# Xiuyu-Li/q-diffusion

Measured on NVIDIA H100. Metric: images_per_sec, higher is better.
Workload: dtype int8 (W4/W8 codes x A8 codes, int32 accumulate; fp32 norms/softmax)

## Files before the change

q-diffusion_b200/csrc/attention_wg.cuh:

```cuda
#pragma once
#include "attention.cuh"
#include "ptx.cuh"

namespace qd {

__device__ __forceinline__ void wgmma_ra_s8s8_n64(uint32_t* d, const uint32_t (&a)[4], uint64_t db, uint32_t scale_d) {
  asm volatile(
      "{\n\t.reg .pred p;\n\t"
      "setp.ne.b32 p, %37, 0;\n\t"
      "wgmma.mma_async.sync.aligned.m64n64k32.s32.s8.s8 "
      "{%0, %1, %2, %3, %4, %5, %6, %7, %8, %9, %10, %11, %12, %13, %14, %15, %16, %17, %18, %19, %20, %21, %22, %23, %24, %25, %26, %27, %28, %29, %30, %31}, {%32, %33, %34, %35}, %36, p;\n\t}\n"
      : "+r"(d[0]), "+r"(d[1]), "+r"(d[2]), "+r"(d[3]), "+r"(d[4]), "+r"(d[5]), "+r"(d[6]), "+r"(d[7]), "+r"(d[8]), "+r"(d[9]), "+r"(d[10]), "+r"(d[11]), "+r"(d[12]), "+r"(d[13]), "+r"(d[14]), "+r"(d[15]), "+r"(d[16]), "+r"(d[17]), "+r"(d[18]), "+r"(d[19]), "+r"(d[20]), "+r"(d[21]), "+r"(d[22]), "+r"(d[23]), "+r"(d[24]), "+r"(d[25]), "+r"(d[26]), "+r"(d[27]), "+r"(d[28]), "+r"(d[29]), "+r"(d[30]), "+r"(d[31])
      : "r"(a[0]), "r"(a[1]), "r"(a[2]), "r"(a[3]), "l"(db), "r"(scale_d));
}
__device__ __forceinline__ void wgmma_ra_u8u8_n64(uint32_t* d, const uint32_t (&a)[4], uint64_t db, uint32_t scale_d) {
  asm volatile(
      "{\n\t.reg .pred p;\n\t"
      "setp.ne.b32 p, %37, 0;\n\t"
      "wgmma.mma_async.sync.aligned.m64n64k32.s32.u8.u8 "
      "{%0, %1, %2, %3, %4, %5, %6, %7, %8, %9, %10, %11, %12, %13, %14, %15, %16, %17, %18, %19, %20, %21, %22, %23, %24, %25, %26, %27, %28, %29, %30, %31}, {%32, %33, %34, %35}, %36, p;\n\t}\n"
      : "+r"(d[0]), "+r"(d[1]), "+r"(d[2]), "+r"(d[3]), "+r"(d[4]), "+r"(d[5]), "+r"(d[6]), "+r"(d[7]), "+r"(d[8]), "+r"(d[9]), "+r"(d[10]), "+r"(d[11]), "+r"(d[12]), "+r"(d[13]), "+r"(d[14]), "+r"(d[15]), "+r"(d[16]), "+r"(d[17]), "+r"(d[18]), "+r"(d[19]), "+r"(d[20]), "+r"(d[21]), "+r"(d[22]), "+r"(d[23]), "+r"(d[24]), "+r"(d[25]), "+r"(d[26]), "+r"(d[27]), "+r"(d[28]), "+r"(d[29]), "+r"(d[30]), "+r"(d[31])
      : "r"(a[0]), "r"(a[1]), "r"(a[2]), "r"(a[3]), "l"(db), "r"(scale_d));
}
__device__ __forceinline__ void wgmma_ra_f16_n64(float* d, const uint32_t (&a)[4], uint64_t db, uint32_t scale_d) {
// ... 97 lines not shown
}
__device__ __forceinline__ void wgmma_ra_u8s8_n96(uint32_t* d, const uint32_t (&a)[4], uint64_t db, uint32_t scale_d) {
  asm volatile(
      "{\n\t.reg .pred p;\n\t"
      "setp.ne.b32 p, %53, 0;\n\t"
      "wgmma.mma_async.sync.aligned.m64n96k32.s32.u8.s8 "
      "{%0, %1, %2, %3, %4, %5, %6, %7, %8, %9, %10, %11, %12, %13, %14, %15, %16, %17, %18, %19, %20, %21, %22, %23, %24, %25, %26, %27, %28, %29, %30, %31, %32, %33, %34, %35, %36, %37, %38, %39, %40, %41, %42, %43, %44, %45, %46, %47}, {%48, %49, %50, %51}, %52, p;\n\t}\n"
      : "+r"(d[0]), "+r"(d[1]), "+r"(d[2]), "+r"(d[3]), "+r"(d[4]), "+r"(d[5]), "+r"(d[6]), "+r"(d[7]), "+r"(d[8]), "+r"(d[9]), "+r"(d[10]), "+r"(d[11]), "+r"(d[12]), "+r"(d[13]), "+r"(d[14]), "+r"(d[15]), "+r"(d[16]), "+r"(d[17]), "+r"(d[18]), "+r"(d[19]), "+r"(d[20]), "+r"(d[21]), "+r"(d[22]), "+r"(d[23]), "+r"(d[24]), "+r"(d[25]), "+r"(d[26]), "+r"(d[27]), "+r"(d[28]), "+r"(d[29]), "+r"(d[30]), "+r"(d[31]), "+r"(d[32]), "+r"(d[33]), "+r"(d[34]), "+r"(d[35]), "+r"(d[36]), "+r"(d[37]), "+r"(d[38]), "+r"(d[39]), "+r"(d[40]), "+r"(d[41]), "+r"(d[42]), "+r"(d[43]), "+r"(d[44]), "+r"(d[45]), "+r"(d[46]), "+r"(d[47])
      : "r"(a[0]), "r"(a[1]), "r"(a[2]), "r"(a[3]), "l"(db), "r"(scale_d));
}
__device__ __forceinline__ void wgmma_ra_u8u8_n112(uint32_t* d, const uint32_t (&a)[4], uint64_t db, uint32_t scale_d) {
  asm volatile(
      "{\n\t.reg .pred p;\n\t"
      "setp.ne.b32 p, %61, 0;\n\t"
      "wgmma.mma_async.sync.aligned.m64n112k32.s32.u8.u8 "
      "{%0, %1, %2, %3, %4, %5, %6, %7, %8, %9, %10, %11, %12, %13, %14, %15, %16, %17, %18, %19, %20, %21, %22, %23, %24, %25, %26, %27, %28, %29, %30, %31, %32, %33, %34, %35, %36, %37, %38, %39, %40, %41, %42, %43, %44, %45, %46, %47, %48, %49, %50, %51, %52, %53, %54, %55}, {%56, %57, %58, %59}, %60, p;\n\t}\n"
      : "+r"(d[0]), "+r"(d[1]), "+r"(d[2]), "+r"(d[3]), "+r"(d[4]), "+r"(d[5]), "+r"(d[6]), "+r"(d[7]), "+r"(d[8]), "+r"(d[9]), "+r"(d[10]), "+r"(d[11]), "+r"(d[12]), "+r"(d[13]), "+r"(d[14]), "+r"(d[15]), "+r"(d[16]), "+r"(d[17]), "+r"(d[18]), "+r"(d[19]), "+r"(d[20]), "+r"(d[21]), "+r"(d[22]), "+r"(d[23]), "+r"(d[24]), "+r"(d[25]), "+r"(d[26]), "+r"(d[27]), "+r"(d[28]), "+r"(d[29]), "+r"(d[30]), "+r"(d[31]), "+r"(d[32]), "+r"(d[33]), "+r"(d[34]), "+r"(d[35]), "+r"(d[36]), "+r"(d[37]), "+r"(d[38]), "+r"(d[39]), "+r"(d[40]), "+r"(d[41]), "+r"(d[42]), "+r"(d[43]), "+r"(d[44]), "+r"(d[45]), "+r"(d[46]), "+r"(d[47]), "+r"(d[48]), "+r"(d[49]), "+r"(d[50]), "+r"(d[51]), "+r"(d[52]), "+r"(d[53]), "+r"(d[54]), "+r"(d[55])
      : "r"(a[0]), "r"(a[1]), "r"(a[2]), "r"(a[3]), "l"(db), "r"(scale_d));
}
__device__ __forceinline__ void wgmma_ra_u8s8_n112(uint32_t* d, const uint32_t (&a)[4], uint64_t db, uint32_t scale_d) {
  asm volatile(
      "{\n\t.reg .pred p;\n\t"
      "setp.ne.b32 p, %61, 0;\n\t"
      "wgmma.mma_async.sync.aligned.m64n112k32.s32.u8.s8 "
      "{%0, %1, %2, %3, %4, %5, %6, %7, %8, %9, %10, %11, %12, %13, %14, %15, %16, %17, %18, %19, %20, %21, %22, %23, %24, %25, %26, %27, %28, %29, %30, %31, %32, %33, %34, %35, %36, %37, %38, %39, %40, %41, %42, %43, %44, %45, %46, %47, %48, %49, %50, %51, %52, %53, %54, %55}, {%56, %57, %58, %59}, %60, p;\n\t}\n"
      : "+r"(d[0]), "+r"(d[1]), "+r"(d[2]), "+r"(d[3]), "+r"(d[4]), "+r"(d[5]), "+r"(d[6]), "+r"(d[7]), "+r"(d[8]), "+r"(d[9]), "+r"(d[10]), "+r"(d[11]), "+r"(d[12]), "+r"(d[13]), "+r"(d[14]), "+r"(d[15]), "+r"(d[16]), "+r"(d[17]), "+r"(d[18]), "+r"(d[19]), "+r"(d[20]), "+r"(d[21]), "+r"(d[22]), "+r"(d[23]), "+r"(d[24]), "+r"(d[25]), "+r"(d[26]), "+r"(d[27]), "+r"(d[28]), "+r"(d[29]), "+r"(d[30]), "+r"(d[31]), "+r"(d[32]), "+r"(d[33]), "+r"(d[34]), "+r"(d[35]), "+r"(d[36]), "+r"(d[37]), "+r"(d[38]), "+r"(d[39]), "+r"(d[40]), "+r"(d[41]), "+r"(d[42]), "+r"(d[43]), "+r"(d[44]), "+r"(d[45]), "+r"(d[46]), "+r"(d[47]), "+r"(d[48]), "+r"(d[49]), "+r"(d[50]), "+r"(d[51]), "+r"(d[52]), "+r"(d[53]), "+r"(d[54]), "+r"(d[55])
      : "r"(a[0]), "r"(a[1]), "r"(a[2]), "r"(a[3]), "l"(db), "r"(scale_d));
}

constexpr int ATW_STAGES = 4;
constexpr int ATW_THREADS = ATT_WARPS * 32;
__host__ __device__ constexpr int atw_nv(int DV) {
  return DV + 8 <= 24 ? 24 : DV + 8 <= 32 ? 32 : DV + 8 <= 48 ? 48 : DV + 8 <= 64 ? 64 : DV + 8 <= 80 ? 80 : DV + 8 <= 96 ? 96 : 112;
}
struct AtwSmem {
  int k_bytes, v_bytes, z_off, bar_off, total;
};
__host__ __device__ inline AtwSmem atw_smem(int P, int NV) {
  AtwSmem l;
  l.k_bytes = (ATT_BN * P + 1023) / 1024 * 1024;
  l.v_bytes = (NV * ATT_BN + 1023) / 1024 * 1024;
  l.z_off = ATW_STAGES * (l.k_bytes + l.v_bytes);
  l.bar_off = l.z_off + ATW_STAGES * ATT_BN * 4;
  l.total = l.bar_off + ATW_STAGES * 8 + ATW_STAGES * 4 + 1024;
  return l;
}
__device__ __forceinline__ uint64_t atw_desc(uint32_t addr, int row_bytes) {
  const uint64_t layout = row_bytes == 128 ? 1 : row_bytes == 64 ? 2 : 3;
  uint64_t d = (uint64_t)((addr & 0x3FFFF) >> 4);
  d |= (uint64_t)1 << 16;
  d |= (uint64_t)((8 * row_bytes) >> 4) << 32;
  d |= layout << 62;
  return d;
}

template <int N, bool VS>
__device__ __forceinline__ void atw_pv(uint32_t* d, const uint32_t (&a)[4], uint64_t db, uint32_t scale_d) {
  if constexpr (VS) {
    if constexpr (N == 24) wgmma_ra_u8s8_n24(d, a, db, scale_d);
    else if constexpr (N == 32) wgmma_ra_u8s8_n32(d, a, db, scale_d);
    else if constexpr (N == 48) wgmma_ra_u8s8_n48(d, a, db, scale_d);
    else if constexpr (N == 64) wgmma_ra_u8s8_n64(d, a, db, scale_d);
    else if constexpr (N == 80) wgmma_ra_u8s8_n80(d, a, db, scale_d);
    else if constexpr (N == 96) wgmma_ra_u8s8_n96(d, a, db, scale_d);
    else wgmma_ra_u8s8_n112(d, a, db, scale_d);
  } else {
    if constexpr (N == 24) wgmma_ra_u8u8_n24(d, a, db, scale_d);
    else if constexpr (N == 32) wgmma_ra_u8u8_n32(d, a, db, scale_d);
    else if constexpr (N == 48) wgmma_ra_u8u8_n48(d, a, db, scale_d);
    else if constexpr (N == 64) wgmma_ra_u8u8_n64(d, a, db, scale_d);
    else if constexpr (N == 80) wgmma_ra_u8u8_n80(d, a, db, scale_d);
    else if constexpr (N == 96) wgmma_ra_u8u8_n96(d, a, db, scale_d);
    else wgmma_ra_u8u8_n112(d, a, db, scale_d);
  }
}

template <int DQ, int DV, bool QK_SIGNED, bool V_SIGNED, bool SM16, bool F16, int MINB>
__global__ void __launch_bounds__(ATW_THREADS, MINB)
qattention_wg_kernel(const __grid_constant__ CUtensorMap tmK, const __grid_constant__ CUtensorMap tmV,
                     const qd_attention_desc p, int P) {
  constexpr int NV = atw_nv(DV);
  constexpr int NKC = DQ / 32;
  constexpr int NDT = DV / 8 + 1;
  constexpr bool MAGIC = DV <= 64;
  constexpr int RB = F16 ? 2 * DV : DV;
  static_assert(!F16 || DV <= 64, "fp16 Q / K operands: d <= 64 keeps |S| below 2^22");
  using SV = att_score_t<F16>;
  extern __shared__ uint8_t atw_raw[];
  uint8_t* smem = atw_raw + (((smem_u32(atw_raw) + 1023u) & ~1023u) - smem_u32(atw_raw));
  const AtwSmem lay = atw_smem(P, NV);
  uint64_t* full = reinterpret_cast<uint64_t*>(smem + lay.bar_off);
  int* released = reinterpret_cast<int*>(full + ATW_STAGES);

  const int warp = threadIdx.x >> 5, lane = threadIdx.x & 31;
  const int g = lane >> 2, t = lane & 3;
  const int bh = blockIdx.y;
  const int b = bh / p.heads, h = bh - b * p.heads;
  const int row0 = blockIdx.x * ATT_BM + warp * 16;
  const int ntiles = (p.Tk + ATT_BN - 1) / ATT_BN;
  const int nloads = 2 * ntiles;
  const bool has_zq = !F16 && p.zq != 0;
  const int* zrk_g = reinterpret_cast<const int*>(p.ws) + (long long)bh * (long long)att_ws_stride(p.Tk);

  for (int i = threadIdx.x; i < ATW_STAGES * (NV - DV) * ATT_BN; i += ATW_THREADS) {
    const int s = i / ((NV - DV) * ATT_BN), r = (i / ATT_BN) % (NV - DV) + DV, c = i % ATT_BN;
    smem[ATW_STAGES * lay.k_bytes + s * lay.v_bytes + r * ATT_BN + c] = r == DV ? 1 : 0;
  }
  if (threadIdx.x == 0) {
    tma_prefetch_desc(&tmK);
    tma_prefetch_desc(&tmV);
    for (int s = 0; s < ATW_STAGES; ++s) {
      mbar_init(&full[s], 1);
      released[s] = 0;
    }
    fence_mbar_init();
  }
  fence_proxy_async();
  __syncthreads();

  auto issue = [&](int L) {
    const int s = L % ATW_STAGES, pass = L / ntiles, tile = L - pass * ntiles;
    const int j0 = tile * ATT_BN;
    const uint32_t bytes = (uint32_t)(ATT_BN * P) + (pass ? (uint32_t)(ATT_BN * DV) : 0u) + (has_zq ? ATT_BN * 4u : 0u);
    mbar_arrive_expect_tx(&full[s], bytes);
    tma_load_2d(smem + s * lay.k_bytes, &tmK, &full[s], h * P, b * p.Tk + j0);
    if (pass) tma_load_2d(smem + ATW_STAGES * lay.k_bytes + s * lay.v_bytes, &tmV, &full[s], j0, bh * DV);
    if (has_zq) bulk_load_1d(smem + lay.z_off + s * ATT_BN * 4, zrk_g + j0, ATT_BN * 4, &full[s]);
  };
  if (threadIdx.x == 0)
    for (int L = 0; L < ATW_STAGES && L < nloads; ++L) issue(L);

  constexpr bool QRELOAD = DV == 48;
  uint32_t qf[NKC][4];
  const uint8_t* qbase = reinterpret_cast<const uint8_t*>(p.q) + (long long)b * p.Tq * p.ld_q + p.q_off + h * p.head_stride_q;
  const uint8_t* q0 = qbase + (long long)min(row0 + g, p.Tq - 1) * p.ld_q;
  const uint8_t* q1 = qbase + (long long)min(row0 + g + 8, p.Tq - 1) * p.ld_q;
  auto load_q = [&]() {
#pragma unroll
    for (int kc = 0; kc < NKC; ++kc) {
      const int c0 = kc * 32 + 4 * t, c1 = c0 + 16;
      qf[kc][0] = c0 < RB ? *reinterpret_cast<const uint32_t*>(q0 + c0) : 0u;
      qf[kc][1] = c0 < RB ? *reinterpret_cast<const uint32_t*>(q1 + c0) : 0u;
      qf[kc][2] = c1 < RB ? *reinterpret_cast<const uint32_t*>(q0 + c1) : 0u;
      qf[kc][3] = c1 < RB ? *reinterpret_cast<const uint32_t*>(q1 + c1) : 0u;
    }
  };
  if constexpr (!QRELOAD) load_q();
  const float c = p.sim_scale * 1.4426950408889634f;
  const bool ragged = (p.Tk % ATT_BN) != 0;
  SV mi0 = att_lowest(SV{}), mi1 = att_lowest(SV{});
  float l0 = 0.f, l1 = 0.f;
  float off0 = 0.f, off1 = 0.f;
  uint32_t olo[NV / 2], ohi[SM16 ? NV / 2 : 1];
  const float pmax = (float)p.p_qmax;
  const QuantK oqk = make_quantk(p.oq);

  auto issue_s = [&](SV (&s)[8][4], int L) {
    const int st = L % ATW_STAGES;
    if constexpr (QRELOAD) load_q();
    mbar_wait(&full[st], (uint32_t)(L / ATW_STAGES) & 1u);
    const uint64_t dK = atw_desc(smem_u32(smem + st * lay.k_bytes), P);
    wgmma_fence();
#pragma unroll
    for (int kc = 0; kc < NKC; ++kc) {
      if constexpr (F16) wgmma_ra_f16_n64(&s[0][0], qf[kc], dK + (uint64_t)(2 * kc), kc ? 1u : 0u);
      else if constexpr (QK_SIGNED) wgmma_ra_s8s8_n64(reinterpret_cast<uint32_t*>(&s[0][0]), qf[kc], dK + (uint64_t)(2 * kc), kc ? 1u : 0u);
      else wgmma_ra_u8u8_n64(reinterpret_cast<uint32_t*>(&s[0][0]), qf[kc], dK + (uint64_t)(2 * kc), kc ? 1u : 0u);
    }
    wgmma_commit();
  };

  auto release = [&](int R) {
    __syncwarp();
    if (lane == 0) {
      const int s = R % ATW_STAGES;
      __threadfence_block();
      const int n = atomicAdd(&released[s], 1);
      if (n == ATT_WARPS * (R / ATW_STAGES + 1) - 1 && R + ATW_STAGES < nloads) {
        __threadfence_block();
        issue(R + ATW_STAGES);
      }
    }
  };

  auto softmax_pv = [&](SV (&sacc)[8][4], int L) {
    const int pass = L >= ntiles ? 1 : 0, tile = L - pass * ntiles, st = L % ATW_STAGES;
    const int j0 = tile * ATT_BN;
    if (L == ntiles) {
      l0 += __shfl_xor_sync(0xffffffffu, l0, 1);
      l0 += __shfl_xor_sync(0xffffffffu, l0, 2);
      l1 += __shfl_xor_sync(0xffffffffu, l1, 1);
      l1 += __shfl_xor_sync(0xffffffffu, l1, 2);
      off0 = -(float)mi0 * c + log2f(1.0f / (l0 * p.delta_w));
      off1 = -(float)mi1 * c + log2f(1.0f / (l1 * p.delta_w));
    }
    const int* sZrk = reinterpret_cast<const int*>(smem + lay.z_off + st * ATT_BN * 4);
    if (has_zq) {
#pragma unroll
      for (int nt = 0; nt < 8; ++nt) {
        const int2 z = *reinterpret_cast<const int2*>(sZrk + 8 * nt + 2 * t);
        sacc[nt][0] -= z.x; sacc[nt][1] -= z.y; sacc[nt][2] -= z.x; sacc[nt][3] -= z.y;
      }
    }
    if (ragged && tile == ntiles - 1) {
      const SV mask = att_mask<MAGIC>(SV{});
#pragma unroll
      for (int nt = 0; nt < 8; ++nt) {
        const int j = j0 + 8 * nt + 2 * t;
        if (j >= p.Tk) { sacc[nt][0] = mask; sacc[nt][2] = mask; }
        if (j + 1 >= p.Tk) { sacc[nt][1] = mask; sacc[nt][3] = mask; }
      }
    }
    if (pass == 0) {
      SV tm0 = sacc[0][0], tm1 = sacc[0][2];
#pragma unroll
      for (int nt = 0; nt < 8; ++nt) {
        tm0 = att_smax(tm0, att_smax(sacc[nt][0], sacc[nt][1]));
        tm1 = att_smax(tm1, att_smax(sacc[nt][2], sacc[nt][3]));
      }
      tm0 = att_smax(tm0, __shfl_xor_sync(0xffffffffu, tm0, 1));
      tm0 = att_smax(tm0, __shfl_xor_sync(0xffffffffu, tm0, 2));
      tm1 = att_smax(tm1, __shfl_xor_sync(0xffffffffu, tm1, 1));
      tm1 = att_smax(tm1, __shfl_xor_sync(0xffffffffu, tm1, 2));
      if (tm0 > mi0) { l0 *= (mi0 == att_lowest(SV{})) ? 0.f : ex2_approx((float)(mi0 - tm0) * c); mi0 = tm0; }
      if (tm1 > mi1) { l1 *= (mi1 == att_lowest(SV{})) ? 0.f : ex2_approx((float)(mi1 - tm1) * c); mi1 = tm1; }
      const float b0 = -(float)mi0 * c, b1 = -(float)mi1 * c;
      float a0 = 0.f, a1 = 0.f;
#pragma unroll
      for (int nt = 0; nt < 8; ++nt) {
        a0 += ex2_approx(fmaf(att_s2f<MAGIC>(sacc[nt][0]), c, b0)) + ex2_approx(fmaf(att_s2f<MAGIC>(sacc[nt][1]), c, b0));
        a1 += ex2_approx(fmaf(att_s2f<MAGIC>(sacc[nt][2]), c, b1)) + ex2_approx(fmaf(att_s2f<MAGIC>(sacc[nt][3]), c, b1));
      }
      l0 += a0;
      l1 += a1;
    } else {
      const uint64_t dV = atw_desc(smem_u32(smem + ATW_STAGES * lay.k_bytes + st * lay.v_bytes), ATT_BN);
      uint32_t plo[2][4], phi[2][4];
#pragma unroll
      for (int kc = 0; kc < 2; ++kc) {
#pragma unroll
        for (int half = 0; half < 2; ++half) {
          const int ntA = 4 * kc + 2 * half, ntB = ntA + 1;
          uint32_t cd[8];
          const SV sv[8] = {sacc[ntA][0], sacc[ntA][1], sacc[ntB][0], sacc[ntB][1],
                            sacc[ntA][2], sacc[ntA][3], sacc[ntB][2], sacc[ntB][3]};
#pragma unroll
          for (int e = 0; e < 8; ++e) {
            const float pr = ex2_approx(fmaf(att_s2f<MAGIC>(sv[e]), c, e < 4 ? off0 : off1));
            cd[e] = __float_as_uint(fminf(pr, pmax) + 12582912.0f);
          }
          plo[kc][2 * half] = __byte_perm(__byte_perm(cd[0], cd[1], 0x0040), __byte_perm(cd[2], cd[3], 0x0040), 0x5410);
          plo[kc][2 * half + 1] = __byte_perm(__byte_perm(cd[4], cd[5], 0x0040), __byte_perm(cd[6], cd[7], 0x0040), 0x5410);
          if constexpr (SM16) {
            phi[kc][2 * half] = __byte_perm(__byte_perm(cd[0], cd[1], 0x0051), __byte_perm(cd[2], cd[3], 0x0051), 0x5410);
            phi[kc][2 * half + 1] = __byte_perm(__byte_perm(cd[4], cd[5], 0x0051), __byte_perm(cd[6], cd[7], 0x0051), 0x5410);
          }
        }
      }
      wgmma_fence();
#pragma unroll
      for (int kc = 0; kc < 2; ++kc) {
        const uint32_t acc = (kc || L > ntiles) ? 1u : 0u;
        atw_pv<NV, V_SIGNED>(olo, plo[kc], dV + (uint64_t)(2 * kc), acc);
        if constexpr (SM16) atw_pv<NV, V_SIGNED>(ohi, phi[kc], dV + (uint64_t)(2 * kc), acc);
      }
      wgmma_commit();
    }
  };

  for (int L = 0; L < nloads; ++L) {
    SV sacc[8][4];
    issue_s(sacc, L);
    wgmma_wait<0>();
#pragma unroll
    for (int i = 0; i < 32; ++i) {
      if constexpr (F16) asm volatile("" : "+f"(sacc[i >> 2][i & 3])::"memory");
      else asm volatile("" : "+r"(sacc[i >> 2][i & 3])::"memory");
    }
    softmax_pv(sacc, L);
    wgmma_wait<0>();
    release(L);
  }
#pragma unroll
  for (int i = 0; i < NV / 2; ++i) asm volatile("" : "+r"(olo[i])::"memory");
#pragma unroll
  for (int i = 0; i < (SM16 ? NV / 2 : 1); ++i) asm volatile("" : "+r"(ohi[i])::"memory");

  float rs0 = (float)(int)olo[4 * (NDT - 1)], rs1 = (float)(int)olo[4 * (NDT - 1) + 2];
  if constexpr (SM16) { rs0 += 256.0f * (float)(int)ohi[4 * (NDT - 1)]; rs1 += 256.0f * (float)(int)ohi[4 * (NDT - 1) + 2]; }
  rs0 = __shfl_sync(0xffffffffu, rs0, lane & ~3);
  rs1 = __shfl_sync(0xffffffffu, rs1, lane & ~3);
  const int r0 = row0 + g, r1 = row0 + g + 8;
  const float z0 = (float)p.zv * rs0, z1 = (float)p.zv * rs1;
#pragma unroll
  for (int nd = 0; nd < NDT - 1; ++nd) {
    const int col = h * DV + 8 * nd + 2 * t;
    float v0 = (float)(int)olo[4 * nd], v1 = (float)(int)olo[4 * nd + 1], v2 = (float)(int)olo[4 * nd + 2], v3 = (float)(int)olo[4 * nd + 3];
    if constexpr (SM16) {
      v0 += 256.0f * (float)(int)ohi[4 * nd]; v1 += 256.0f * (float)(int)ohi[4 * nd + 1];
      v2 += 256.0f * (float)(int)ohi[4 * nd + 2]; v3 += 256.0f * (float)(int)ohi[4 * nd + 3];
    }
    const float y0 = (v0 - z0) * p.out_scale, y1 = (v1 - z0) * p.out_scale;
    const float y2 = (v2 - z1) * p.out_scale, y3 = (v3 - z1) * p.out_scale;
    if (p.out) {
      if (r0 < p.Tq) *reinterpret_cast<float2*>(p.out + ((long long)b * p.Tq + r0) * p.ld_out + col) = make_float2(y0, y1);
      if (r1 < p.Tq) *reinterpret_cast<float2*>(p.out + ((long long)b * p.Tq + r1) * p.ld_out + col) = make_float2(y2, y3);
    }
    if (p.out_q) {
      uint8_t* oq = reinterpret_cast<uint8_t*>(p.out_q);
      if (r0 < p.Tq)
        *reinterpret_cast<uint16_t*>(oq + ((long long)b * p.Tq + r0) * p.ld_out_q + col) =
            (uint16_t)(quant_code(y0, oqk) | (quant_code(y1, oqk) << 8));
      if (r1 < p.Tq)
        *reinterpret_cast<uint16_t*>(oq + ((long long)b * p.Tq + r1) * p.ld_out_q + col) =
            (uint16_t)(quant_code(y2, oqk) | (quant_code(y3, oqk) << 8));
    }
  }
}

}
```

q-diffusion_b200/csrc/engine.cu:

```cuda
#include <cuda.h>
#include <cuda_runtime.h>
#include <cudaTypedefs.h>

#include <atomic>
#include <cstdarg>
#include <cstdio>
#include <cstdlib>
#include <cstring>
#include <mutex>
#include <new>
#include <utility>
#include <vector>

#include "../../include/qdiff_b200.h"
#include "attention.cuh"
#include "attention_wg.cuh"
#include "elem.cuh"
#include "gemm_i8.cuh"

namespace {

thread_local char g_err[512] = "";
std::atomic<long long> g_launches{0};
constexpr int kMaxDevices = 64;
// ... 681 lines not shown
}

int validate_im2col(const qd_im2col_desc& d) {
  if (!d.src || !d.dst) return fail(QD_ERR_BAD_ARG, "im2col: null arg");
  if (d.B <= 0 || d.H <= 0 || d.W <= 0 || d.C <= 0 || d.Ho <= 0 || d.Wo <= 0 || d.stride <= 0)
    return fail(QD_ERR_BAD_ARG, "im2col: empty geometry");
  if (d.ld_dst < 9 * d.C) return fail(QD_ERR_BAD_ARG, "im2col: ld_dst too small");
  return QD_OK;
}

int launch_im2col(const qd_im2col_desc& d, cudaStream_t s) {
  if (int rc = validate_im2col(d)) return rc;
  if (im2col_vec(d)) {
    launch_k(qd::im2col_vec_kernel, grid_for((long long)d.B * d.Ho * d.Wo * 9 * (d.C / 16), 256), 256, 0, s, d);
    return check_launch("im2col_vec_kernel");
  }
  const long long total = (long long)d.B * d.Ho * d.Wo * d.ld_dst;
  launch_k(qd::im2col_kernel, grid_for(total, 256), 256, 0, s, d);
  return check_launch("im2col_kernel");
}

template <int DQ, int DV, bool QS, bool VS, bool S16, bool F16>
int launch_attention_inst(const qd_attention_desc& d, cudaStream_t s) {
  constexpr int MINB = (DV <= 48) ? 2 : 1;
  auto kern = qd::qattention_kernel<DQ, DV, QS, VS, S16, MINB, F16>;
  static std::atomic<unsigned long long> optin{0};
  if (int rc = ensure_smem_optin(kern, 200 * 1024, optin, "attention")) return rc;
  const bool zrk = !F16 && d.zq != 0;
  const qd::AttSmemLayout lay = qd::att_smem_layout(DQ, DV, d.Tk, zrk);
  if (lay.total > 200 * 1024) return fail(QD_ERR_UNSUPPORTED, "attention: Tk=%d needs %d B of shared memory", d.Tk, lay.total);
  if (zrk) {
    if (!d.ws) return fail(QD_ERR_BAD_ARG, "attention: workspace required when zq != 0");
    const int tk_pad = qd::att_ws_stride(d.Tk);
    launch_k(qd::att_krowsum_kernel<QS>, grid_for((long long)d.B * d.heads * tk_pad, 256), 256, 0, s, d, tk_pad, 0, 0);
    int rc = check_launch("att_krowsum_kernel");
    if (rc) return rc;
  }
  dim3 grid((d.Tq + qd::ATT_BM - 1) / qd::ATT_BM, d.B * d.heads);
  launch_k(kern, grid, qd::ATT_WARPS * 32, lay.total, s, d);
  return check_launch("qattention_kernel");
}

template <int DQ, int DV, bool F16 = false>
int launch_attention_t(const qd_attention_desc& d, cudaStream_t s) {
  const bool qs = d.q_signed != 0, vs = d.v_signed != 0, s16 = d.sm_bits > 8;
  if (qs && vs && s16) return launch_attention_inst<DQ, DV, true, true, true, F16>(d, s);
  if (qs && vs && !s16) return launch_attention_inst<DQ, DV, true, true, false, F16>(d, s);
  if (!qs && !vs && s16) return launch_attention_inst<DQ, DV, false, false, true, F16>(d, s);
  if (!qs && !vs && !s16) return launch_attention_inst<DQ, DV, false, false, false, F16>(d, s);
  return fail(QD_ERR_UNSUPPORTED, "attention: mixed signedness q=%d v=%d", d.q_signed, d.v_signed);
}

template <int DQ, int DV, bool QS, bool VS, bool S16>
int launch_attention_smallk_inst(const qd_attention_desc& d, cudaStream_t s) {
  constexpr int NKV = 3;
  auto kern = qd::qattention_smallk_kernel<DQ, DV, QS, VS, S16, NKV>;
  const int spw = d.Tq >= 2048 ? 4 : (d.Tq >= 512 ? 2 : 1);
  const int slabs = (d.Tq + 15) / 16;
  dim3 grid((slabs + spw * qd::ATS_WARPS - 1) / (spw * qd::ATS_WARPS), d.B * d.heads);
  launch_k(kern, grid, qd::ATS_WARPS * 32, qd::ats_smem_bytes<DQ, DV, NKV>(), s, d, spw);
  return check_launch("qattention_smallk_kernel");
}

template <int DQ, int DV>
int launch_attention_smallk(const qd_attention_desc& d, cudaStream_t s) {
  const bool qs = d.q_signed != 0, vs = d.v_signed != 0, s16 = d.sm_bits > 8;
  if (qs && vs && s16) return launch_attention_smallk_inst<DQ, DV, true, true, true>(d, s);
  if (qs && vs && !s16) return launch_attention_smallk_inst<DQ, DV, true, true, false>(d, s);
  if (!qs && !vs && s16) return launch_attention_smallk_inst<DQ, DV, false, false, true>(d, s);
  if (!qs && !vs && !s16) return launch_attention_smallk_inst<DQ, DV, false, false, false>(d, s);
  return fail(QD_ERR_UNSUPPORTED, "attention: mixed signedness q=%d v=%d", d.q_signed, d.v_signed);
}

bool attention_wg_eligible(const qd_attention_desc& d) {
  static const int forced_mma = [] { const char* e = getenv("QDIFF_ATTENTION"); return (e && !strcmp(e, "mma")) ? 1 : 0; }();
  if (forced_mma) return false;
  const int P = d.head_stride_q, rb = d.qk_f16 ? 2 * d.d : d.d;
  if (d.d != 16 && d.d != 24 && d.d != 32 && d.d != 40 && d.d != 48 && d.d != 64 && d.d != 80 && d.d != 96) return false;
  if (d.qk_f16 && d.d > 64) return false;
  if ((P != 32 && P != 64 && P != 128) || P < rb || d.head_stride_k != P) return false;
  if (d.q_off != 0 || d.k_off != 0 || (d.ld_k & 15) || (((uintptr_t)d.k) & 15) || (((uintptr_t)d.vt) & 15)) return false;
  if (d.v_off != 0 || d.head_stride_v != d.d || d.v_batch_stride != (long long)d.heads * d.d * d.ld_vt) return false;
  if (d.zq != 0 && !d.qk_f16 && !d.ws) return false;
  return true;
}

template <int DQ, int DV, bool QS, bool VS, bool S16, bool F16>
int launch_attention_wg_inst(const qd_attention_desc& d, cudaStream_t s) {
  constexpr int MINB = DV <= 40 ? 2 : 1;
  auto kern = qd::qattention_wg_kernel<DQ, DV, QS, VS, S16, F16, MINB>;
  const int P = d.head_stride_q;
  const qd::AtwSmem lay = qd::atw_smem(P, qd::atw_nv(DV));
  static std::atomic<unsigned long long> optin{0};
  if (int rc = ensure_smem_optin(kern, 227 * 1024, optin, "attention_wg")) return rc;
  CUtensorMap tmK, tmV;
  {
    cuuint64_t dims[2] = {(cuuint64_t)d.ld_k, (cuuint64_t)d.B * d.Tk};
    cuuint64_t strides[1] = {(cuuint64_t)d.ld_k};
    cuuint32_t box[2] = {(cuuint32_t)P, (cuuint32_t)qd::ATT_BN};
    if (int rc = encode_u8_map(&tmK, d.k, 2, dims, strides, box, P)) return rc;
  }
  {
    cuuint64_t dims[2] = {(cuuint64_t)d.ld_vt, (cuuint64_t)d.B * d.heads * d.d};
    cuuint64_t strides[1] = {(cuuint64_t)d.ld_vt};
    cuuint32_t box[2] = {(cuuint32_t)qd::ATT_BN, (cuuint32_t)d.d};
    if (int rc = encode_u8_map(&tmV, d.vt, 2, dims, strides, box, 64)) return rc;
  }
  if (!F16 && d.zq != 0) {
    const int tk_pad = qd::att_ws_stride(d.Tk);
    launch_k(qd::att_krowsum_kernel<QS>, grid_for((long long)d.B * d.heads * tk_pad, 256), 256, 0, s, d, tk_pad, 0, 0);
    if (int rc = check_launch("att_krowsum_kernel")) return rc;
  }
  dim3 grid((d.Tq + qd::ATT_BM - 1) / qd::ATT_BM, d.B * d.heads);
  launch_k(kern, grid, qd::ATW_THREADS, lay.total, s, tmK, tmV, d, P);
  return check_launch("qattention_wg_kernel");
}

template <int DQ, int DV, bool F16>
int launch_attention_wg_t(const qd_attention_desc& d, cudaStream_t s) {
  const bool qs = d.q_signed != 0, vs = d.v_signed != 0, s16 = d.sm_bits > 8;
  if (qs && vs && s16) return launch_attention_wg_inst<DQ, DV, true, true, true, F16>(d, s);
  if (qs && vs && !s16) return launch_attention_wg_inst<DQ, DV, true, true, false, F16>(d, s);
  if (!qs && !vs && s16) return launch_attention_wg_inst<DQ, DV, false, false, true, F16>(d, s);
  if (!qs && !vs && !s16) return launch_attention_wg_inst<DQ, DV, false, false, false, F16>(d, s);
  return fail(QD_ERR_UNSUPPORTED, "attention: mixed signedness q=%d v=%d", d.q_signed, d.v_signed);
}

int launch_attention_wg(const qd_attention_desc& d, cudaStream_t s) {
  if (d.qk_f16) {
    switch (d.d) {
      case 16: return launch_attention_wg_t<32, 16, true>(d, s);
      case 24: return launch_attention_wg_t<64, 24, true>(d, s);
      case 32: return launch_attention_wg_t<64, 32, true>(d, s);
      case 40: return launch_attention_wg_t<96, 40, true>(d, s);
      case 48: return launch_attention_wg_t<96, 48, true>(d, s);
      default: return launch_attention_wg_t<128, 64, true>(d, s);
    }
  }
  switch (d.d) {
    case 16: return launch_attention_wg_t<32, 16, false>(d, s);
    case 24: return launch_attention_wg_t<32, 24, false>(d, s);
    case 32: return launch_attention_wg_t<32, 32, false>(d, s);
    case 40: return launch_attention_wg_t<64, 40, false>(d, s);
    case 48: return launch_attention_wg_t<64, 48, false>(d, s);
    case 64: return launch_attention_wg_t<64, 64, false>(d, s);
    case 80: return launch_attention_wg_t<96, 80, false>(d, s);
    default: return launch_attention_wg_t<96, 96, false>(d, s);
  }
}

int validate_attention(const qd_attention_desc& d) {
  if (!d.q || !d.k || !d.vt || (!d.out && !d.out_q)) return fail(QD_ERR_BAD_ARG, "attention: null arg");
  if (d.out_q && (d.ld_out_q & 1)) return fail(QD_ERR_UNSUPPORTED, "attention: ld_out_q");
  if (d.q_signed != d.k_signed) return fail(QD_ERR_UNSUPPORTED, "attention: q/k signedness differ");
  if (d.zw != 0) return fail(QD_ERR_UNSUPPORTED, "attention: softmax zero point must be 0 (got %d)", d.zw);
  if (d.sm_bits != 8 && d.sm_bits != 16) return fail(QD_ERR_UNSUPPORTED, "attention: sm_bits %d", d.sm_bits);
  if (!(d.sim_scale > 0.f)) return fail(QD_ERR_UNSUPPORTED, "attention: sim_scale must be positive (got %g)", d.sim_scale);
  if (!d.qk_f16 && d.d > 64 &&
      (2147483648.0 - 65025.0 * d.d) * d.sim_scale * 1.4426950408889634 < 128.0 + fmax(0.0, -log2((double)d.delta_w)))
    return fail(QD_ERR_UNSUPPORTED, "attention: sim_scale %g too small to mask the keys beyond Tk at d = %d", d.sim_scale, d.d);
  if (d.ld_vt % 16 || d.ld_vt < d.Tk) return fail(QD_ERR_BAD_ARG, "attention: ld_vt");
  if ((d.q_off | d.head_stride_q | (int)d.ld_q) & 3) return fail(QD_ERR_UNSUPPORTED, "attention: q needs 4-byte alignment");
  if ((d.k_off | d.head_stride_k | (int)d.ld_k | d.d) & 7) return fail(QD_ERR_UNSUPPORTED, "attention: k rows need 8-byte alignment");
  if (d.out && (d.ld_out % 2)) return fail(QD_ERR_UNSUPPORTED, "attention: ld_out");
  return QD_OK;
}
// ... 315 lines not shown
```

Measured before the change: 4.113.

## Convert int scores to float via magic-number bias and split softmax passes

Replaces the per-element int-to-float conversion of attention scores with a magic-constant add and reinterpret. The zero-point correction moves into the float domain instead of integer subtraction. The two-pass loop (max/sum pass, then PV pass) is split into separate loops, so the first pass releases stages early and carries no output accumulators, which may ease register pressure. Eligibility gains a zero-point range check, and large zq falls back to the other path.

```diff
diff --git a/q-diffusion_b200/csrc/attention_wg.cuh b/q-diffusion_b200/csrc/attention_wg.cuh
--- a/q-diffusion_b200/csrc/attention_wg.cuh
+++ b/q-diffusion_b200/csrc/attention_wg.cuh
@@ -203,10 +203,11 @@
   constexpr int NV = atw_nv(DV);
   constexpr int NKC = DQ / 32;
   constexpr int NDT = DV / 8 + 1;
-  constexpr bool MAGIC = DV <= 64;
   constexpr int RB = F16 ? 2 * DV : DV;
   static_assert(!F16 || DV <= 64, "fp16 Q / K operands: d <= 64 keeps |S| below 2^22");
-  using SV = att_score_t<F16>;
+  static_assert(DV <= 96, "8-bit codes: the raw scores must stay below 2^23 (unsigned) / 2^22 (signed)");
+  using SV = std::conditional_t<F16, float, uint32_t>;
+  constexpr uint32_t MB = QK_SIGNED ? 0x4B400000u : 0x4B000000u;
   extern __shared__ uint8_t atw_raw[];
   uint8_t* smem = atw_raw + (((smem_u32(atw_raw) + 1023u) & ~1023u) - smem_u32(atw_raw));
   const AtwSmem lay = atw_smem(P, NV);
@@ -269,12 +270,8 @@
   if constexpr (!QRELOAD) load_q();
   const float c = p.sim_scale * 1.4426950408889634f;
   const bool ragged = (p.Tk % ATT_BN) != 0;
-  SV mi0 = att_lowest(SV{}), mi1 = att_lowest(SV{});
+  float mi0 = -INFINITY, mi1 = -INFINITY;
   float l0 = 0.f, l1 = 0.f;
-  float off0 = 0.f, off1 = 0.f;
-  uint32_t olo[NV / 2], ohi[SM16 ? NV / 2 : 1];
-  const float pmax = (float)p.p_qmax;
-  const QuantK oqk = make_quantk(p.oq);
 
   auto issue_s = [&](SV (&s)[8][4], int L) {
     const int st = L % ATW_STAGES;
@@ -285,10 +282,39 @@
 #pragma unroll
     for (int kc = 0; kc < NKC; ++kc) {
       if constexpr (F16) wgmma_ra_f16_n64(&s[0][0], qf[kc], dK + (uint64_t)(2 * kc), kc ? 1u : 0u);
-      else if constexpr (QK_SIGNED) wgmma_ra_s8s8_n64(reinterpret_cast<uint32_t*>(&s[0][0]), qf[kc], dK + (uint64_t)(2 * kc), kc ? 1u : 0u);
-      else wgmma_ra_u8u8_n64(reinterpret_cast<uint32_t*>(&s[0][0]), qf[kc], dK + (uint64_t)(2 * kc), kc ? 1u : 0u);
+      else if constexpr (QK_SIGNED) wgmma_ra_s8s8_n64(&s[0][0], qf[kc], dK + (uint64_t)(2 * kc), kc ? 1u : 0u);
+      else wgmma_ra_u8u8_n64(&s[0][0], qf[kc], dK + (uint64_t)(2 * kc), kc ? 1u : 0u);
     }
     wgmma_commit();
+  };
+  auto scores = [&](SV (&s)[8][4], float (&f)[8][4], int L) {
+    wgmma_fence_regs(reinterpret_cast<SV (&)[32]>(s));
+    const int tile = L % ntiles, st = L % ATW_STAGES;
+    if constexpr (F16) {
+#pragma unroll
+      for (int i = 0; i < 32; ++i) f[i >> 2][i & 3] = s[i >> 2][i & 3];
+    } else {
+      const uint32_t* sZrk = reinterpret_cast<const uint32_t*>(smem + lay.z_off + st * ATT_BN * 4);
+#pragma unroll
+      for (int nt = 0; nt < 8; ++nt) {
+        float z0 = __uint_as_float(MB), z1 = z0;
+        if (has_zq) {
+          const uint2 z = *reinterpret_cast<const uint2*>(sZrk + 8 * nt + 2 * t);
+          z0 = __uint_as_float(z.x + MB);
+          z1 = __uint_as_float(z.y + MB);
+        }
+        f[nt][0] = __uint_as_float(s[nt][0] + MB) - z0; f[nt][1] = __uint_as_float(s[nt][1] + MB) - z1;
+        f[nt][2] = __uint_as_float(s[nt][2] + MB) - z0; f[nt][3] = __uint_as_float(s[nt][3] + MB) - z1;
+      }
+    }
+    if (ragged && tile == ntiles - 1) {
+#pragma unroll
+      for (int nt = 0; nt < 8; ++nt) {
+        const int j = tile * ATT_BN + 8 * nt + 2 * t;
+        if (j >= p.Tk) { f[nt][0] = -INFINITY; f[nt][2] = -INFINITY; }
+        if (j + 1 >= p.Tk) { f[nt][1] = -INFINITY; f[nt][3] = -INFINITY; }
+      }
+    }
   };
 
   auto release = [&](int R) {
@@ -304,101 +330,85 @@
     }
   };
 
-  auto softmax_pv = [&](SV (&sacc)[8][4], int L) {
-    const int pass = L >= ntiles ? 1 : 0, tile = L - pass * ntiles, st = L % ATW_STAGES;
-    const int j0 = tile * ATT_BN;
-    if (L == ntiles) {
-      l0 += __shfl_xor_sync(0xffffffffu, l0, 1);
-      l0 += __shfl_xor_sync(0xffffffffu, l0, 2);
-      l1 += __shfl_xor_sync(0xffffffffu, l1, 1);
-      l1 += __shfl_xor_sync(0xffffffffu, l1, 2);
-      off0 = -(float)mi0 * c + log2f(1.0f / (l0 * p.delta_w));
-      off1 = -(float)mi1 * c + log2f(1.0f / (l1 * p.delta_w));
-    }
-    const int* sZrk = reinterpret_cast<const int*>(smem + lay.z_off + st * ATT_BN * 4);
-    if (has_zq) {
-#pragma unroll
-      for (int nt = 0; nt < 8; ++nt) {
-        const int2 z = *reinterpret_cast<const int2*>(sZrk + 8 * nt + 2 * t);
-        sacc[nt][0] -= z.x; sacc[nt][1] -= z.y; sacc[nt][2] -= z.x; sacc[nt][3] -= z.y;
-      }
-    }
-    if (ragged && tile == ntiles - 1) {
-      const SV mask = att_mask<MAGIC>(SV{});
-#pragma unroll
-      for (int nt = 0; nt < 8; ++nt) {
-        const int j = j0 + 8 * nt + 2 * t;
-        if (j >= p.Tk) { sacc[nt][0] = mask; sacc[nt][2] = mask; }
-        if (j + 1 >= p.Tk) { sacc[nt][1] = mask; sacc[nt][3] = mask; }
-      }
-    }
-    if (pass == 0) {
-      SV tm0 = sacc[0][0], tm1 = sacc[0][2];
-#pragma unroll
-      for (int nt = 0; nt < 8; ++nt) {
-        tm0 = att_smax(tm0, att_smax(sacc[nt][0], sacc[nt][1]));
-        tm1 = att_smax(tm1, att_smax(sacc[nt][2], sacc[nt][3]));
-      }
-      tm0 = att_smax(tm0, __shfl_xor_sync(0xffffffffu, tm0, 1));
-      tm0 = att_smax(tm0, __shfl_xor_sync(0xffffffffu, tm0, 2));
-      tm1 = att_smax(tm1, __shfl_xor_sync(0xffffffffu, tm1, 1));
-      tm1 = att_smax(tm1, __shfl_xor_sync(0xffffffffu, tm1, 2));
-      if (tm0 > mi0) { l0 *= (mi0 == att_lowest(SV{})) ? 0.f : ex2_approx((float)(mi0 - tm0) * c); mi0 = tm0; }
-      if (tm1 > mi1) { l1 *= (mi1 == att_lowest(SV{})) ? 0.f : ex2_approx((float)(mi1 - tm1) * c); mi1 = tm1; }
-      const float b0 = -(float)mi0 * c, b1 = -(float)mi1 * c;
-      float a0 = 0.f, a1 = 0.f;
-#pragma unroll
-      for (int nt = 0; nt < 8; ++nt) {
-        a0 += ex2_approx(fmaf(att_s2f<MAGIC>(sacc[nt][0]), c, b0)) + ex2_approx(fmaf(att_s2f<MAGIC>(sacc[nt][1]), c, b0));
-        a1 += ex2_approx(fmaf(att_s2f<MAGIC>(sacc[nt][2]), c, b1)) + ex2_approx(fmaf(att_s2f<MAGIC>(sacc[nt][3]), c, b1));
-      }
-      l0 += a0;
-      l1 += a1;
-    } else {
-      const uint64_t dV = atw_desc(smem_u32(smem + ATW_STAGES * lay.k_bytes + st * lay.v_bytes), ATT_BN);
-      uint32_t plo[2][4], phi[2][4];
-#pragma unroll
-      for (int kc = 0; kc < 2; ++kc) {
-#pragma unroll
-        for (int half = 0; half < 2; ++half) {
-          const int ntA = 4 * kc + 2 * half, ntB = ntA + 1;
-          uint32_t cd[8];
-          const SV sv[8] = {sacc[ntA][0], sacc[ntA][1], sacc[ntB][0], sacc[ntB][1],
-                            sacc[ntA][2], sacc[ntA][3], sacc[ntB][2], sacc[ntB][3]};
-#pragma unroll
-          for (int e = 0; e < 8; ++e) {
-            const float pr = ex2_approx(fmaf(att_s2f<MAGIC>(sv[e]), c, e < 4 ? off0 : off1));
-            cd[e] = __float_as_uint(fminf(pr, pmax) + 12582912.0f);
-          }
-          plo[kc][2 * half] = __byte_perm(__byte_perm(cd[0], cd[1], 0x0040), __byte_perm(cd[2], cd[3], 0x0040), 0x5410);
-          plo[kc][2 * half + 1] = __byte_perm(__byte_perm(cd[4], cd[5], 0x0040), __byte_perm(cd[6], cd[7], 0x0040), 0x5410);
-          if constexpr (SM16) {
-            phi[kc][2 * half] = __byte_perm(__byte_perm(cd[0], cd[1], 0x0051), __byte_perm(cd[2], cd[3], 0x0051), 0x5410);
-            phi[kc][2 * half + 1] = __byte_perm(__byte_perm(cd[4], cd[5], 0x0051), __byte_perm(cd[6], cd[7], 0x0051), 0x5410);
-          }
-        }
-      }
-      wgmma_fence();
-#pragma unroll
-      for (int kc = 0; kc < 2; ++kc) {
-        const uint32_t acc = (kc || L > ntiles) ? 1u : 0u;
-        atw_pv<NV, V_SIGNED>(olo, plo[kc], dV + (uint64_t)(2 * kc), acc);
-        if constexpr (SM16) atw_pv<NV, V_SIGNED>(ohi, phi[kc], dV + (uint64_t)(2 * kc), acc);
-      }
-      wgmma_commit();
-    }
-  };
-
-  for (int L = 0; L < nloads; ++L) {
+  for (int L = 0; L < ntiles; ++L) {
     SV sacc[8][4];
     issue_s(sacc, L);
     wgmma_wait<0>();
-#pragma unroll
-    for (int i = 0; i < 32; ++i) {
-      if constexpr (F16) asm volatile("" : "+f"(sacc[i >> 2][i & 3])::"memory");
-      else asm volatile("" : "+r"(sacc[i >> 2][i & 3])::"memory");
-    }
-    softmax_pv(sacc, L);
+    float f[8][4];
+    scores(sacc, f, L);
+    release(L);
+    float tm0 = f[0][0], tm1 = f[0][2];
+#pragma unroll
+    for (int nt = 0; nt < 8; ++nt) {
+      tm0 = fmaxf(tm0, fmaxf(f[nt][0], f[nt][1]));
+      tm1 = fmaxf(tm1, fmaxf(f[nt][2], f[nt][3]));
+    }
+    tm0 = fmaxf(tm0, __shfl_xor_sync(0xffffffffu, tm0, 1));
+    tm0 = fmaxf(tm0, __shfl_xor_sync(0xffffffffu, tm0, 2));
+    tm1 = fmaxf(tm1, __shfl_xor_sync(0xffffffffu, tm1, 1));
+    tm1 = fmaxf(tm1, __shfl_xor_sync(0xffffffffu, tm1, 2));
+    if (tm0 > mi0) { l0 *= (mi0 == -INFINITY) ? 0.f : ex2_approx((mi0 - tm0) * c); mi0 = tm0; }
+    if (tm1 > mi1) { l1 *= (mi1 == -INFINITY) ? 0.f : ex2_approx((mi1 - tm1) * c); mi1 = tm1; }
+    const float b0 = -mi0 * c, b1 = -mi1 * c;
+    float a0 = 0.f, a1 = 0.f;
+#pragma unroll
+    for (int nt = 0; nt < 8; ++nt) {
+      a0 += ex2_approx(fmaf(f[nt][0], c, b0)) + ex2_approx(fmaf(f[nt][1], c, b0));
+      a1 += ex2_approx(fmaf(f[nt][2], c, b1)) + ex2_approx(fmaf(f[nt][3], c, b1));
+    }
+    l0 += a0;
+    l1 += a1;
+  }
+
+  l0 += __shfl_xor_sync(0xffffffffu, l0, 1);
+  l0 += __shfl_xor_sync(0xffffffffu, l0, 2);
+  l1 += __shfl_xor_sync(0xffffffffu, l1, 1);
+  l1 += __shfl_xor_sync(0xffffffffu, l1, 2);
+  const float off0 = -mi0 * c + log2f(1.0f / (l0 * p.delta_w));
+  const float off1 = -mi1 * c + log2f(1.0f / (l1 * p.delta_w));
+  const float pmax = (float)p.p_qmax;
+  const QuantK oqk = make_quantk(p.oq);
+  auto codes = [&](SV (&s)[8][4], uint32_t (&cw)[8][4], int L) {
+    float f[8][4];
+    scores(s, f, L);
+#pragma unroll
+    for (int i = 0; i < 32; ++i)
+      cw[i >> 2][i & 3] = __float_as_uint(fminf(ex2_approx(fmaf(f[i >> 2][i & 3], c, (i & 2) ? off1 : off0)), pmax) + 12582912.0f);
+  };
+  uint32_t plo[2][4], phi[2][4];
+  auto pack = [&](const uint32_t (&cw)[8][4]) {
+#pragma unroll
+    for (int kc = 0; kc < 2; ++kc) {
+#pragma unroll
+      for (int half = 0; half < 2; ++half) {
+        const int ntA = 4 * kc + 2 * half, ntB = ntA + 1;
+        const uint32_t cd[8] = {cw[ntA][0], cw[ntA][1], cw[ntB][0], cw[ntB][1], cw[ntA][2], cw[ntA][3], cw[ntB][2], cw[ntB][3]};
+        plo[kc][2 * half] = __byte_perm(__byte_perm(cd[0], cd[1], 0x0040), __byte_perm(cd[2], cd[3], 0x0040), 0x5410);
+        plo[kc][2 * half + 1] = __byte_perm(__byte_perm(cd[4], cd[5], 0x0040), __byte_perm(cd[6], cd[7], 0x0040), 0x5410);
+        if constexpr (SM16) {
+          phi[kc][2 * half] = __byte_perm(__byte_perm(cd[0], cd[1], 0x0051), __byte_perm(cd[2], cd[3], 0x0051), 0x5410);
+          phi[kc][2 * half + 1] = __byte_perm(__byte_perm(cd[4], cd[5], 0x0051), __byte_perm(cd[6], cd[7], 0x0051), 0x5410);
+        }
+      }
+    }
+  };
+  uint32_t olo[NV / 2], ohi[SM16 ? NV / 2 : 1];
+  for (int L = ntiles; L < nloads; ++L) {
+    SV sacc[8][4];
+    uint32_t cw[8][4];
+    issue_s(sacc, L);
+    wgmma_wait<0>();
+    codes(sacc, cw, L);
+    pack(cw);
+    const uint64_t dV = atw_desc(smem_u32(smem + ATW_STAGES * lay.k_bytes + (L % ATW_STAGES) * lay.v_bytes), ATT_BN);
+    wgmma_fence();
+#pragma unroll
+    for (int kc = 0; kc < 2; ++kc) {
+      const uint32_t acc = (kc || L > ntiles) ? 1u : 0u;
+      atw_pv<NV, V_SIGNED>(olo, plo[kc], dV + (uint64_t)(2 * kc), acc);
+      if constexpr (SM16) atw_pv<NV, V_SIGNED>(ohi, phi[kc], dV + (uint64_t)(2 * kc), acc);
+    }
+    wgmma_commit();
     wgmma_wait<0>();
     release(L);
   }
diff --git a/q-diffusion_b200/csrc/engine.cu b/q-diffusion_b200/csrc/engine.cu
--- a/q-diffusion_b200/csrc/engine.cu
+++ b/q-diffusion_b200/csrc/engine.cu
@@ -787,6 +787,7 @@
   if (d.q_off != 0 || d.k_off != 0 || (d.ld_k & 15) || (((uintptr_t)d.k) & 15) || (((uintptr_t)d.vt) & 15)) return false;
   if (d.v_off != 0 || d.head_stride_v != d.d || d.v_batch_stride != (long long)d.heads * d.d * d.ld_vt) return false;
   if (d.zq != 0 && !d.qk_f16 && !d.ws) return false;
+  if (!d.qk_f16 && (d.zq > 255 || d.zq < (d.q_signed ? -255 : 0))) return false;
   return true;
 }
 
```

New measurement: 4.348 (median of 6 runs). 1.06x the previous value.
